# yuvalH9/UMERegRobust

Hardware: AMD Instinct MI355X
Metric: registration_pairs_per_s (higher is better)
Workload: dtype f32

## Files before the change

umeregrobust_amd/csrc/match_dev.h:

```cpp
#pragma once
#include "common.h"
#include "qlayout.h"

namespace umereg {

using f32x16 = __attribute__((ext_vector_type(16))) float;
using half8 = __attribute__((ext_vector_type(8))) _Float16;
using f32x2 = __attribute__((ext_vector_type(2))) float;

constexpr int kDistWaves = 4;

constexpr int kRegionCap = 512;
constexpr int kMaxSplits = 64;
constexpr unsigned int kShareMask = 0x8000808bu;

struct MatchScratch {
    unsigned int* rowlim;
    unsigned int* cnt;
    unsigned int* cand;
    int splits;
    unsigned int share_mask;
    int force_exhaustive;
    const int* ord1;
    const int* ord2;
    unsigned long long* stats;
};

constexpr int kCoarseTA = 2;
constexpr int kCoarseRows = kCoarseTA * 8;
constexpr int kCoarseWG = kCoarseRows * kDistWaves;

constexpr int kPK = 33;
constexpr int kPWaves = 8;
constexpr int kPRows = 32;
constexpr int kPWG = kPRows * kPWaves;
constexpr int kPRegionCap = 1024;

inline size_t qa_bytes(int n1) { return align_up((size_t)n1, 128) * 128 * sizeof(float); }
inline size_t qb_bytes(int n2) { return align_up((size_t)n2, 32) * 128 * sizeof(float); }
struct CoarsePlan {
    int n_ablk, n_blocks, n_btiles, splits, tiles_per_split;
    int sub_tiles, sub_tps, sub_splits;
};
struct MatchOpts {
    int variant = 0;
    int splits = 0;
    long long share_mask = -1;
    int exhaustive = 0;
};
inline int resolve_opts(const umereg_match_opts* o, MatchOpts& m, const char* who)
{
    m = MatchOpts();
    if (!o) return UMEREG_OK;
    UMEREG_REQUIRE(o->variant == 0 || o->variant == 1, "%s: unknown matcher variant %d (0 = Q-form, 1 = P-form)", who, (int)o->variant);
    UMEREG_REQUIRE(o->splits >= 0 && o->force_exhaustive >= 0, "%s: negative matcher option", who);
    UMEREG_REQUIRE(o->share_mask <= 0xffffffffll, "%s: share_mask does not fit 32 bits", who);
    UMEREG_REQUIRE(o->reserved == 0, "%s: umereg_match_opts.reserved must be 0 (got %d)", who, (int)o->reserved);
    m.variant = o->variant;
    m.splits = o->splits;
    m.share_mask = o->share_mask;
    m.exhaustive = o->force_exhaustive ? 1 : 0;
    return UMEREG_OK;
}
inline bool use_pform(const MatchOpts& o) { return o.variant == 1; }
constexpr int kNumCU = 256;
#ifndef UMEREG_COARSE_PHASES
#define UMEREG_COARSE_PHASES 3
#endif
constexpr int kMinSplitTiles = 4;
constexpr int kLeadMinTiles = 64;

inline CoarsePlan coarse_plan(int n1, int n2, const MatchOpts& o)
{
    CoarsePlan p;
    p.n_btiles = (n2 + 31) / 32;
    int splits;
    if (use_pform(o)) {
        p.n_ablk = (n1 + kPWG - 1) / kPWG;
        p.n_blocks = p.n_ablk * kPWaves;
        splits = kNumCU / p.n_ablk;
    } else {
        p.n_ablk = (n1 + kCoarseWG - 1) / kCoarseWG;
        p.n_blocks = p.n_ablk * kDistWaves;
        splits = (2560 + p.n_ablk - 1) / p.n_ablk;
    }
    p.sub_tiles = p.sub_tps = p.sub_splits = 0;
    if (UMEREG_COARSE_PHASES >= 2 && !use_pform(o) && o.splits <= 0 && p.n_btiles >= kLeadMinTiles) {
        const int n_sub = (n2 + kSubStride - 1) / kSubStride;
        p.sub_tiles = (n_sub + 31) / 32;
        int s1 = 4 * kNumCU / p.n_ablk;
        s1 = s1 < 1 ? 1 : (s1 > 16 ? 16 : s1);
        s1 = s1 > p.sub_tiles / kMinSplitTiles ? p.sub_tiles / kMinSplitTiles : s1;
        p.sub_tps = (p.sub_tiles + s1 - 1) / s1;
        p.sub_splits = (p.sub_tiles + p.sub_tps - 1) / p.sub_tps;
        const int bulk = p.n_btiles - p.sub_tiles;
        int s2 = splits > kMaxSplits - 16 ? kMaxSplits - 16 : splits;
        s2 = s2 > bulk / kMinSplitTiles ? bulk / kMinSplitTiles : s2;
        p.tiles_per_split = (bulk + s2 - 1) / s2;
        p.splits = p.sub_splits + (bulk + p.tiles_per_split - 1) / p.tiles_per_split;
        return p;
    }
    if (o.splits > 0) splits = o.splits;
    if (splits > kMaxSplits) splits = kMaxSplits;
    if (splits > p.n_btiles) splits = p.n_btiles;
    if (splits < 1) splits = 1;
    p.tiles_per_split = (p.n_btiles + splits - 1) / splits;
    p.splits = (p.n_btiles + p.tiles_per_split - 1) / p.tiles_per_split;
    return p;
}
inline size_t region_cap(const MatchOpts& o) { return use_pform(o) ? (size_t)kPRegionCap : (size_t)kRegionCap; }
inline size_t cand_bytes(int n1, const CoarsePlan& p, const MatchOpts& o)
{
    return align_up(((size_t)n1 + (size_t)p.n_blocks * p.splits * (1 + region_cap(o))) * sizeof(unsigned int), 256);
}
inline size_t pfrag_bytes(const CoarsePlan& p, const MatchOpts& o)
{
    return use_pform(o) ? ((size_t)p.n_blocks + (size_t)p.n_btiles) * kPK * 64 * sizeof(half8) : 0;
}
#ifndef UMEREG_COARSE_STATS
#define UMEREG_COARSE_STATS 0
#endif
constexpr size_t kStatsBytes = UMEREG_COARSE_STATS ? 256 : 0;
inline size_t match_scratch_bytes(int n1, int n2, const MatchOpts& o = MatchOpts())
{
    const CoarsePlan p = coarse_plan(n1, n2, o);
    return cand_bytes(n1, p, o) + pfrag_bytes(p, o) + kStatsBytes;
}

inline int match_args(const void* Q1_rows_h, const void* Q2_cols_h, int n1, int n2, void* scratch, size_t scratch_bytes,
                      const MatchOpts& o, const char* who)
{
    UMEREG_REQUIRE(Q1_rows_h && Q2_cols_h, "%s: null basis pointer", who);
    UMEREG_REQUIRE(n1 > 0 && n2 > 0, "%s: n1, n2 must be positive (got %d, %d)", who, n1, n2);
    UMEREG_REQUIRE(n2 < (1 << 27), "%s: n2 must be below 2^27 (got %d)", who, n2);
    UMEREG_REQUIRE(((uintptr_t)Q1_rows_h & 15) == 0 && ((uintptr_t)Q2_cols_h & 15) == 0, "%s: misaligned basis pointer", who);
    if (int rc = check_device()) return rc;
    if (!scratch || scratch_bytes < match_scratch_bytes(n1, n2, o) || ((uintptr_t)scratch & 15)) {
        set_error("%s: scratch too small or misaligned (%zu < %zu)", who, scratch_bytes, match_scratch_bytes(n1, n2, o));
        return UMEREG_EWORKSPACE;
    }
    return UMEREG_OK;
}

inline MatchScratch carve_scratch(void* scratch, int n1, const CoarsePlan& p, const MatchOpts& o, const int* ord1 = nullptr,
                                  const int* ord2 = nullptr)
{
    MatchScratch ms;
    ms.rowlim = (unsigned int*)scratch;
    ms.cnt = ms.rowlim + n1;
    ms.cand = ms.cnt + (size_t)p.n_blocks * p.splits;
    ms.splits = p.splits;
    ms.share_mask = o.share_mask >= 0 ? (unsigned int)o.share_mask : kShareMask;
    ms.force_exhaustive = o.exhaustive;
    ms.ord1 = ord1;
    ms.ord2 = ord2;
    ms.stats = UMEREG_COARSE_STATS ? (unsigned long long*)((char*)scratch + cand_bytes(n1, p, o) + pfrag_bytes(p, o)) : nullptr;
    return ms;
}
inline half8* pfrag_rows(void* scratch, int n1, const CoarsePlan& p, const MatchOpts& o) { return (half8*)((char*)scratch + cand_bytes(n1, p, o)); }
inline half8* pfrag_cols(void* scratch, int n1, const CoarsePlan& p, const MatchOpts& o) { return pfrag_rows(scratch, n1, p, o) + (size_t)p.n_blocks * kPK * 64; }

int launch_orthobasis_pair(const float* ume1, int n1, int layout1, float* Q1, const float* ume2, int n2, int layout2, float* Q2,
                           hipStream_t st, const int* order1 = nullptr, const int* order2 = nullptr);
int match_refine_f16(const void* Q1_rows_h, const void* Q2_cols_h, int n1, int n2, const void* scratch, size_t scratch_bytes,
                     int64_t* match_idx, float* match_dist, const umereg_match_opts* opts, const int* order1, const int* order2,
                     void* stream);
int match_f16r_ordered(const float* ume1, const float* ume2, int n1, int n2, const int* order1, const int* order2,
                       int64_t* match_idx, float* match_dist, void* workspace, size_t workspace_bytes,
                       const umereg_match_opts* opts, void* stream);

}
```

umeregrobust_amd/csrc/match_f16r.hip:

```cpp
#include <type_traits>

#include "common.h"
#include "match_dev.h"
#include "qlayout.h"

namespace umereg {

constexpr float kCoarseMargin = 0.03125f + 0.0009765625f;
constexpr float kCoarseTermMax = 1.00390625f;
#ifndef UMEREG_COARSE_EXIT
#define UMEREG_COARSE_EXIT 3
#endif

__device__ __forceinline__ float group32_max(float v)
{
    int x = __float_as_int(v);
    x = __float_as_int(fmaxf(__int_as_float(x), __int_as_float(__builtin_amdgcn_mov_dpp(x, 0xB1, 0xf, 0xf, true))));
    x = __float_as_int(fmaxf(__int_as_float(x), __int_as_float(__builtin_amdgcn_mov_dpp(x, 0x4E, 0xf, 0xf, true))));
    x = __float_as_int(fmaxf(__int_as_float(x), __int_as_float(__builtin_amdgcn_mov_dpp(x, 0x141, 0xf, 0xf, true))));
    x = __float_as_int(fmaxf(__int_as_float(x), __int_as_float(__builtin_amdgcn_mov_dpp(x, 0x140, 0xf, 0xf, true))));
    x = __float_as_int(fmaxf(__int_as_float(x), __int_as_float(__builtin_amdgcn_ds_swizzle(x, 0x401F))));
    return __int_as_float(x);
}

#ifndef UMEREG_COARSE_ABLATE
#define UMEREG_COARSE_ABLATE 0
#endif
#ifndef UMEREG_COARSE_TPS
#define UMEREG_COARSE_TPS 2
#endif
constexpr int kCoarseTPS = UMEREG_COARSE_TPS;

__global__ __launch_bounds__(kWave* kDistWaves, 2) void ume_coarse_h_kernel(
    const half8* __restrict__ Afrag, const half8* __restrict__ Bfrag, int n1, int n2, int n_ablk, int tile_lo, int tile_mid, int tile_hi,
    int lead_tps, int lead_splits, int tiles_per_split, int sp0, MatchScratch ms)
{
    __shared__ half8 ldsB[2][kCoarseTPS * 512];
    const int wave = __builtin_amdgcn_readfirstlane(threadIdx.x >> 6);
    const int lane = lane_id();
    const int ablk = blockIdx.x % n_ablk;
    const int spl = blockIdx.x / n_ablk;
    const int sp = sp0 + spl;
    const bool lead = spl < lead_splits;
    const int jt0 = lead ? tile_lo + spl * lead_tps : tile_mid + (spl - lead_splits) * tiles_per_split;
    const int jt1 = lead ? min(jt0 + lead_tps, tile_mid) : min(jt0 + tiles_per_split, tile_hi);
    const int h = lane >> 5;
    const int i_base = ablk * kCoarseWG + wave * kCoarseRows;

    half8 a[kCoarseTA][2];
#pragma unroll
    for (int t = 0; t < kCoarseTA; ++t)
#pragma unroll
        for (int s = 0; s < 2; ++s)
            a[t][s] = Afrag[((((size_t)(ablk * (kCoarseWG / 8) + wave * kCoarseTA + t)) * 2 + s) * 2 + 0) * 64 + lane];

    int lim[kCoarseTA][4];
    unsigned int seen[kCoarseTA][4];
#pragma unroll
    for (int t = 0; t < kCoarseTA; ++t)
#pragma unroll
        for (int g = 0; g < 4; ++g) {
            const int i = i_base + t * 8 + 2 * g + h;
            seen[t][g] = __hip_atomic_load(ms.rowlim + min(i, n1 - 1), __ATOMIC_RELAXED, __HIP_MEMORY_SCOPE_AGENT);
            lim[t][g] = i < n1 ? max(__float_as_int(1.0e-30f), (int)seen[t][g]) : __float_as_int(3.0e38f);
        }
#pragma unroll
    for (int t = 0; t < kCoarseTA; ++t)
#pragma unroll
        for (int s = 0; s < 2; ++s) asm volatile("" ::"v"(a[t][s]));

    const int blk = ablk * kDistWaves + wave;
    unsigned int* const region = ms.cand + ((size_t)blk * ms.splits + sp) * kRegionCap;
    int qn = 0;
    auto share = [&](bool reload) __attribute__((always_inline)) {
#pragma unroll
        for (int t = 0; t < kCoarseTA; ++t)
#pragma unroll
            for (int g = 0; g < 4; ++g) {
                const float v = group32_max(__int_as_float(lim[t][g]));
                const int i = i_base + t * 8 + 2 * g + h;
                if ((lane & 31) == 0 && i < n1 && __float_as_uint(v) > seen[t][g]) atomicMax(ms.rowlim + i, __float_as_uint(v));
                lim[t][g] = max(__float_as_int(v), (int)seen[t][g]);
            }
        if (reload) {
#pragma unroll
            for (int t = 0; t < kCoarseTA; ++t)
#pragma unroll
                for (int g = 0; g < 4; ++g) {
                    const int i = min(i_base + t * 8 + 2 * g + h, n1 - 1);
                    seen[t][g] = __hip_atomic_load(ms.rowlim + i, __ATOMIC_RELAXED, __HIP_MEMORY_SCOPE_AGENT);
                }
        }
    };

    half8 st[kCoarseTPS][2];
    const int c0 = threadIdx.x, c1 = 256 + threadIdx.x;
    const int src0 = ((c0 >> 6) * 2) * 64 + (c0 & 63), src1 = ((c1 >> 6) * 2) * 64 + (c1 & 63);
    auto gload = [&](int jg) __attribute__((always_inline)) {
#pragma unroll
        for (int q = 0; q < kCoarseTPS; ++q) {
            const int jt = min(jg + q, jt1 - 1);
            st[q][0] = Bfrag[(size_t)jt * 1024 + src0];
            st[q][1] = Bfrag[(size_t)jt * 1024 + src1];
        }
    };
    auto lstore = [&](int buf) __attribute__((always_inline)) {
#pragma unroll
        for (int q = 0; q < kCoarseTPS; ++q) {
            ldsB[buf][q * 512 + c0] = st[q][0];
            ldsB[buf][q * 512 + c1] = st[q][1];
        }
    };
    if (jt0 < jt1) {
        gload(jt0);
        lstore(0);
    }
    if (jt0 + kCoarseTPS < jt1) gload(jt0 + kCoarseTPS);
    __syncthreads();
    int cur = 0;
    auto share_point = [&](const int jt) __attribute__((always_inline)) {
        const int kt = jt - jt0;
        if ((ms.share_mask >> (kt < 31 ? kt : 31)) & 1u) {
            if (kt < 31 || (kt & 31) == 31) share(true);
        }
    };
#if UMEREG_COARSE_STATS
    unsigned int n_stop1 = 0, n_stop2 = 0;
#endif
    auto hopeless = [&](const float (&sc)[kCoarseTA][4], const int cols) __attribute__((always_inline)) {
        float d = sc[0][0] - __int_as_float(lim[0][0]);
#pragma unroll
        for (int t = 0; t < kCoarseTA; ++t)
#pragma unroll
            for (int g = 0; g < 4; ++g) d = fmaxf(d, sc[t][g] - __int_as_float(lim[t][g]));
        const bool stop = __builtin_amdgcn_ballot_w64(!(d < -(float)(4 - cols) * kCoarseTermMax)) == 0ull;
        return (UMEREG_COARSE_ABLATE & 16) ? true : stop;
    };
    auto filter = [&](const int jt, const float (&sc)[kCoarseTA][4]) __attribute__((always_inline)) {
        if (UMEREG_COARSE_ABLATE & 2) {
#pragma unroll
            for (int t = 0; t < kCoarseTA; ++t)
#pragma unroll
                for (int g = 0; g < 4; ++g) lim[t][g] = max(lim[t][g], __float_as_int(sc[t][g]));
            return;
        }
#pragma unroll
        for (int t = 0; t < kCoarseTA; ++t)
#pragma unroll
            for (int g = 0; g < 4; ++g) lim[t][g] = max(lim[t][g], __float_as_int(sc[t][g] - kCoarseMargin));
        share_point(jt);
        unsigned long long hit[kCoarseTA][4], any = 0;
#pragma unroll
        for (int t = 0; t < kCoarseTA; ++t)
#pragma unroll
            for (int g = 0; g < 4; ++g) {
                hit[t][g] = __builtin_amdgcn_ballot_w64(sc[t][g] >= __int_as_float(lim[t][g]));
                any |= hit[t][g];
            }
        if (__builtin_popcountll(any) > 8) {
#pragma unroll
            for (int t = 0; t < kCoarseTA; ++t)
#pragma unroll
                for (int g = 0; g < 4; ++g) lim[t][g] = __float_as_int(group32_max(__int_as_float(lim[t][g])));
            any = 0;
#pragma unroll
            for (int t = 0; t < kCoarseTA; ++t)
#pragma unroll
                for (int g = 0; g < 4; ++g) {
                    hit[t][g] = __builtin_amdgcn_ballot_w64(sc[t][g] >= __int_as_float(lim[t][g]));
                    any |= hit[t][g];
                }
        }
        if (any) {
            const unsigned int j = (unsigned int)(jt * 32 + (lane & 31));
#pragma unroll
            for (int t = 0; t < kCoarseTA; ++t)
#pragma unroll
                for (int g = 0; g < 4; ++g) {
                    const unsigned long long mask = hit[t][g];
                    if (mask) {
                        const int pos = qn + mbcnt(mask);
                        if (((mask >> lane) & 1ull) && pos < kRegionCap)
                            region[pos] = ((unsigned int)(t * 8 + 2 * g + h) << 27) | j;
                        qn += __builtin_popcountll(mask);
                    }
                }
        }
    };
    auto tile = [&](const int jt, const int q) __attribute__((always_inline)) {
        const half8* const lB = &ldsB[cur][q * 512];
        float sc[kCoarseTA][4];
        auto products = [&](const int b, f32x16 (&cc)[kCoarseTA]) __attribute__((always_inline)) {
            const half8 b0 = (UMEREG_COARSE_ABLATE & 8) ? a[0][0] : lB[(b * 2 + 0) * 64 + lane];
            const half8 b1 = (UMEREG_COARSE_ABLATE & 8) ? a[0][1] : lB[(b * 2 + 1) * 64 + lane];
            if (UMEREG_COARSE_ABLATE & 4) {
#pragma unroll
                for (int t = 0; t < kCoarseTA; ++t)
#pragma unroll
                    for (int e = 0; e < 16; ++e) cc[t][e] = (float)b0[e & 7] + (float)b1[(e + t) & 7];
            } else {
#pragma unroll
                for (int t = 0; t < kCoarseTA; ++t) cc[t] = __builtin_amdgcn_mfma_f32_32x32x16_f16(a[t][0], b0, f32x16{0}, 0, 0, 0);
#pragma unroll
                for (int t = 0; t < kCoarseTA; ++t) cc[t] = __builtin_amdgcn_mfma_f32_32x32x16_f16(a[t][1], b1, cc[t], 0, 0, 0);
            }
        };
        auto squares = [&](const int b, const f32x16 (&cc)[kCoarseTA]) __attribute__((always_inline)) {
#pragma unroll
            for (int t = 0; t < kCoarseTA; ++t)
#pragma unroll
                for (int g = 0; g < 4; ++g) {
                    if (UMEREG_COARSE_ABLATE & 1) {
                        sc[t][g] = b == 0 ? cc[t][4 * g] : sc[t][g] + cc[t][4 * g + 1];
                        continue;
                    }
                    float acc = b == 0 ? cc[t][4 * g] * cc[t][4 * g] : fmaf(cc[t][4 * g], cc[t][4 * g], sc[t][g]);
                    acc = fmaf(cc[t][4 * g + 1], cc[t][4 * g + 1], acc);
                    acc = fmaf(cc[t][4 * g + 2], cc[t][4 * g + 2], acc);
                    sc[t][g] = fmaf(cc[t][4 * g + 3], cc[t][4 * g + 3], acc);
                }
        };
        constexpr bool kTest1 = (UMEREG_COARSE_EXIT & 1) && !(UMEREG_COARSE_ABLATE & 15), kTest2 = (UMEREG_COARSE_EXIT & 2) && !(UMEREG_COARSE_ABLATE & 15);
        constexpr bool kAhead = (UMEREG_COARSE_EXIT & 4) != 0;
        f32x16 c0[kCoarseTA], c1[kCoarseTA];
        products(0, c0);
        if (kAhead || !kTest1) products(1, c1);
        squares(0, c0);
        if (kTest1 && hopeless(sc, 1)) {
#if UMEREG_COARSE_STATS
            ++n_stop1;
#endif
            share_point(jt);
            return;
        }
        if (!kAhead && kTest1) products(1, c1);
        squares(1, c1);
        if (kTest2 && hopeless(sc, 2)) {
#if UMEREG_COARSE_STATS
            ++n_stop2;
#endif
            share_point(jt);
            return;
        }
#pragma unroll
        for (int b = 2; b < 4; ++b) {
            f32x16 cc[kCoarseTA];
            products(b, cc);
            squares(b, cc);
        }
        filter(jt, sc);
    };
    for (int jg = jt0; jg < jt1; jg += kCoarseTPS) {
#pragma unroll
        for (int q = 0; q < kCoarseTPS; ++q)
            if (jg + q < jt1) tile(jg + q, q);
        if (jg + kCoarseTPS < jt1) lstore(cur ^ 1);
        if (jg + 2 * kCoarseTPS < jt1) gload(jg + 2 * kCoarseTPS);
        __syncthreads();
        cur ^= 1;
    }
    share(false);
    if (lane == 0) ms.cnt[(size_t)blk * ms.splits + sp] = (unsigned int)qn;
#if UMEREG_COARSE_STATS
    if (lane == 0) {
        atomicAdd(ms.stats + 0, (unsigned long long)max(jt1 - jt0, 0));
        atomicAdd(ms.stats + 1, (unsigned long long)n_stop1);
        atomicAdd(ms.stats + 2, (unsigned long long)n_stop2);
        atomicAdd(ms.stats + 3, (unsigned long long)qn);
    }
#endif
}

constexpr float kCoarseMarginP = 0.009765625f;
constexpr int kPDepth = 5;
constexpr int kQsStride = 33;

__global__ __launch_bounds__(256) void pform_pack_kernel(const _Float16* __restrict__ Ah, const _Float16* __restrict__ Bh, int n1,
                                                         int n2, int tiles1, int tiles2, half8* __restrict__ PA,
                                                         half8* __restrict__ PB)
{
    __shared__ float4 qs[32 * kQsStride];
    const int side = blockIdx.y, tile = blockIdx.x;
    if (tile >= (side ? tiles2 : tiles1)) return;
    const int n = side ? n2 : n1;
    const _Float16* const Q = side ? Bh : Ah;
    half8* const P = (side ? PB : PA) + (size_t)tile * kPK * 64;
    const int tid = threadIdx.x;
    if (tile * 32 >= n) {
        for (int o = tid; o < kPK * 64; o += 256) P[o] = half8{0};
        return;
    }
    float* const qf = reinterpret_cast<float*>(qs);
    for (int c = tid; c < 512; c += 256) {
        const int kp = c & 31, a = (c >> 5) & 3, k8 = c >> 7;
        const int i = tile * 32 + kp;
        half8 vh = half8{0}, vl = half8{0};
        if (i < n) {
            const size_t off0 = side ? hoff_cols(i, a, k8 * 8, 0) : hoff_rows(i, a, k8 * 8, 0);
            const size_t off1 = side ? hoff_cols(i, a, k8 * 8, 1) : hoff_rows(i, a, k8 * 8, 1);
            vh = *reinterpret_cast<const half8*>(Q + off0);
            vl = *reinterpret_cast<const half8*>(Q + off1);
        }
#pragma unroll
        for (int x = 0; x < 8; ++x) qf[(kp * kQsStride + k8 * 8 + x) * 4 + a] = (float)vh[x] + (float)vl[x];
    }
    __syncthreads();
    for (int o = tid; o < kPK * 64; o += 256) {
        const int ks = o >> 6, l = o & 63, kp = l & 31, c = ks * 2 + (l >> 5);
        half8 out = half8{0};
        if (c < 66) {
            const int d = c < 64 ? c >> 2 : 16, u0 = c < 64 ? (c & 3) * 8 : (c - 64) * 8;
            const float w = d == 0 ? 1.0f : 1.41421356237f;
#pragma unroll
            for (int e = 0; e < 8; ++e) {
                const float4 qu = qs[kp * kQsStride + u0 + e], qv = qs[kp * kQsStride + ((u0 + e + d) & 31)];
                out[e] = (_Float16)(w * fmaf(qu.x, qv.x, fmaf(qu.y, qv.y, fmaf(qu.z, qv.z, qu.w * qv.w))));
            }
        }
        P[o] = out;
    }
}

__global__ __launch_bounds__(kWave* kPWaves, 2) void ume_coarse_p_kernel(const half8* __restrict__ PA, const half8* __restrict__ PB,
                                                                        int n1, int n2, int n_ablk, int n_btiles,
                                                                        int tiles_per_split, MatchScratch ms)
{
    __shared__ half8 ldsB[3][kPK * 64];
    __shared__ __attribute__((aligned(16))) unsigned int seenL[kPWaves][32];
    const int wave = __builtin_amdgcn_readfirstlane(threadIdx.x >> 6);
    const int lane = lane_id();
    const int ablk = blockIdx.x % n_ablk;
    const int sp = blockIdx.x / n_ablk;
    const int jt0 = sp * tiles_per_split;
    const int jt1 = min(jt0 + tiles_per_split, n_btiles);
    const int h = lane >> 5;
    const int atile = ablk * kPWaves + wave;
    const int i_base = atile * 32;

    half8 a[kPK];
#pragma unroll
    for (int ks = 0; ks < kPK; ++ks) a[ks] = PA[((size_t)atile * kPK + ks) * 64 + lane];

    int lim[16];
#pragma unroll
    for (int r = 0; r < 16; ++r) {
        const int i = i_base + (r >> 2) * 8 + h * 4 + (r & 3);
        lim[r] = __float_as_int(i < n1 ? 1.0e-30f : 3.0e38f);
    }
    int qn = 0;
    auto fetch_seen = [&]() __attribute__((always_inline)) {
        if (lane < 32)
            __builtin_amdgcn_global_load_lds((const __attribute__((address_space(1))) void*)(ms.rowlim + min(i_base + lane, n1 - 1)),
                                             (__attribute__((address_space(3))) void*)(&seenL[wave][0]), 4, 0, 16 );
    };
    auto share = [&](bool reload) __attribute__((always_inline)) {
        asm volatile("s_waitcnt vmcnt(0)" ::: "memory");
#pragma unroll
        for (int g = 0; g < 4; ++g) {
            const uint4 sv = *reinterpret_cast<const uint4*>(&seenL[wave][g * 8 + h * 4]);
            const unsigned int seen[4] = {sv.x, sv.y, sv.z, sv.w};
#pragma unroll
            for (int e = 0; e < 4; ++e) {
                const int r = g * 4 + e;
                const float v = group32_max(__int_as_float(lim[r]));
                const int i = i_base + g * 8 + h * 4 + e;
                if ((lane & 31) == 0 && i < n1 && __float_as_uint(v) > seen[e]) atomicMax(ms.rowlim + i, __float_as_uint(v));
                lim[r] = max(__float_as_int(v), (int)seen[e]);
            }
        }
        if (reload) fetch_seen();
    };
    unsigned int* const region = ms.cand + ((size_t)atile * ms.splits + sp) * kPRegionCap;
    auto tile_candidates = [&](const f32x16& cc, const int jt) __attribute__((always_inline)) {
        unsigned long long any = 0;
#pragma unroll
        for (int r = 0; r < 16; ++r) any |= __builtin_amdgcn_ballot_w64(cc[r] >= __int_as_float(lim[r]));
        if (__builtin_popcountll(any) > 8) {
#pragma unroll
            for (int r = 0; r < 16; ++r) lim[r] = __float_as_int(group32_max(__int_as_float(lim[r])));
        }
        const unsigned int j = (unsigned int)(jt * 32 + (lane & 31));
#pragma unroll
        for (int r = 0; r < 16; ++r) {
            const unsigned long long mask = __builtin_amdgcn_ballot_w64(cc[r] >= __int_as_float(lim[r]));
            if (mask) {
                const int pos = qn + mbcnt(mask);
                if (((mask >> lane) & 1ull) && pos < kPRegionCap)
                    region[pos] = ((unsigned int)((r >> 2) * 8 + h * 4 + (r & 3)) << 27) | j;
                qn += __builtin_popcountll(mask);
            }
        }
    };

    auto stage = [&](int jt, int buf) __attribute__((always_inline)) {
        const half8* const src = PB + (size_t)jt * kPK * 64 + lane;
#pragma unroll
        for (int q = 0; q < (kPK + kPWaves / 2 - 1) / (kPWaves / 2); ++q) {
            const int f = q * (kPWaves / 2) + wave;
            if (f < kPK)
                __builtin_amdgcn_global_load_lds((const __attribute__((address_space(1))) void*)(src + f * 64),
                                                 (__attribute__((address_space(3))) void*)(&ldsB[buf][f * 64]), 16, 0, 0);
        }
    };
    auto limits = [&](const f32x16& cc, unsigned int& fl) __attribute__((always_inline)) {
#pragma unroll
        for (int r = 0; r < 16; ++r) {
            lim[r] = max(lim[r], __float_as_int(cc[r] - kCoarseMarginP));
            fl = __builtin_amdgcn_alignbit(fl, __float_as_int(cc[r] - __int_as_float(lim[r])), 31);
        }
    };
    auto bookkeeping = [&](const f32x16& cc, const unsigned int fl, const int jp) __attribute__((always_inline)) {
        const int kt = jp - jt0;
        if ((ms.share_mask >> (kt < 31 ? kt : 31)) & 1u) {
            if (kt < 31 || (kt & 31) == 31) share(true);
        }
        unsigned int hits = ~fl & 0xffffu;
        unsigned long long mask = __builtin_amdgcn_ballot_w64(hits != 0);
        if (__builtin_popcountll(mask) > 8) {
            tile_candidates(cc, jp);
        } else {
            const unsigned int j = (unsigned int)(jp * 32 + (lane & 31));
            while (mask) {
                if (hits) {
                    const int k = 31 - __builtin_clz(hits);
                    hits &= ~(1u << k);
                    const int r = 15 - k;
                    const int pos = qn + mbcnt(mask);
                    if (pos < kPRegionCap) region[pos] = ((unsigned int)((r >> 2) * 8 + h * 4 + (r & 3)) << 27) | j;
                }
                qn += __builtin_popcountll(mask);
                mask = __builtin_amdgcn_ballot_w64(hits != 0);
            }
        }
    };
    auto mfma_panel = [&](const int buf, f32x16& acc, const f32x16& prev, unsigned int& fl, auto interleave) __attribute__((always_inline)) {
        const half8* const lb = &ldsB[buf][lane];
        half8 b[kPDepth];
#pragma unroll
        for (int q = 0; q < kPDepth; ++q) b[q] = lb[q * 64];
        __builtin_amdgcn_sched_barrier(0);
#pragma unroll
        for (int ks = 0; ks < kPK; ++ks) {
            if (ks >= 1 && ks - 1 + kPDepth < kPK) b[(ks - 1) % kPDepth] = lb[(ks - 1 + kPDepth) * 64];
            __builtin_amdgcn_sched_barrier(0);
            if (ks == 0) asm volatile("v_mfma_f32_32x32x16_f16 %0, %1, %2, 0" : "=v"(acc) : "a"(a[ks]), "v"(b[ks % kPDepth]));
            else if (ks < 32) asm volatile("v_mfma_f32_32x32x16_f16 %0, %1, %2, %0" : "+v"(acc) : "a"(a[ks]), "v"(b[ks % kPDepth]));
            else asm volatile("v_mfma_f32_32x32x16_f16 %0, %1, %2, %0" : "+v"(acc) : "v"(a[ks]), "v"(b[ks % kPDepth]));
            if (decltype(interleave)::value && ks < 32 && (ks & 1) == 0) {
                const int r = ks >> 1;
                lim[r] = max(lim[r], __float_as_int(prev[r] - kCoarseMarginP));
                fl = __builtin_amdgcn_alignbit(fl, __float_as_int(prev[r] - __int_as_float(lim[r])), 31);
                asm volatile("" : "+v"(fl), "+v"(lim[r]));
            }
            __builtin_amdgcn_sched_barrier(0);
        }
        asm volatile("s_nop 15\n\ts_nop 15\n\ts_nop 15\n\ts_nop 15" : "+v"(acc) : : "memory");
    };
    const bool young = wave >= kPWaves / 2;
    auto panel = [&](const int jt, f32x16& acc, f32x16& prev) __attribute__((always_inline)) {
        const int buf = (jt - jt0) % 3;
        unsigned int fl = ~0u;
        if (young) {
            if (jt > jt0) {
                limits(prev, fl);
                bookkeeping(prev, fl, jt - 1);
            }
            mfma_panel(buf, acc, prev, fl, std::false_type{});
        } else {
            mfma_panel(buf, acc, prev, fl, std::true_type{});
            asm volatile("s_waitcnt vmcnt(0)" ::: "memory");
            if (jt > jt0) bookkeeping(prev, fl, jt - 1);
            if (jt + 2 < jt1) stage(jt + 2, (buf + 2) % 3);
        }
        asm volatile("s_waitcnt lgkmcnt(0)\n\ts_barrier" ::: "memory");
    };
    if (!young) {
        if (jt0 < jt1) stage(jt0, 0);
        if (jt0 + 1 < jt1) stage(jt0 + 1, 1);
    }
    fetch_seen();
    asm volatile("s_waitcnt vmcnt(0)" ::: "memory");
    __syncthreads();
    f32x16 accA, accB;
    accA = accB = f32x16{-1.0f};
    int jt = jt0;
    for (; jt + 1 < jt1; jt += 2) {
        panel(jt, accA, accB);
        panel(jt + 1, accB, accA);
    }
    if (jt < jt1) {
        panel(jt, accA, accB);
        accB = accA;
    }
    if (jt0 < jt1) {
        unsigned int fl = ~0u;
        limits(accB, fl);
        bookkeeping(accB, fl, jt1 - 1);
    }
    share(false);
    if (lane == 0) ms.cnt[(size_t)atile * ms.splits + sp] = (unsigned int)qn;
}

constexpr int kQiStride = 130;

template <int kRows, int kCap>
__global__ __launch_bounds__(256, 4) void match_refine_kernel(const _Float16* __restrict__ Ah,
                                                           const _Float16* __restrict__ Bh, int n1, int n2,
                                                           MatchScratch ms, int64_t* __restrict__ idx,
                                                           float* __restrict__ dist)
{
    constexpr int kCoarseRows = kRows, kRegionCap = kCap;
    __shared__ double qi[kCoarseRows * kQiStride];
    __shared__ unsigned long long best[kCoarseRows];
    __shared__ unsigned int offs[kWave + 1];
    __shared__ int overflow;
    const int blk = blockIdx.x;
    const int i0 = blk * kCoarseRows;
    const int tid = threadIdx.x;
    if (tid < kWave) {
        const unsigned int c = tid < ms.splits ? ms.cnt[(size_t)blk * ms.splits + tid] : 0u;
        const bool ovf = c > (unsigned int)kRegionCap;
        unsigned int incl = min(c, (unsigned int)kRegionCap);
#pragma unroll
        for (int d = 1; d < kWave; d <<= 1) {
            const unsigned int up = (unsigned int)__shfl_up((int)incl, d, kWave);
            if (tid >= d) incl += up;
        }
        offs[tid + 1] = incl;
        const bool any_ovf = __builtin_amdgcn_ballot_w64(ovf) != 0ull;
        if (tid == 0) {
            offs[0] = 0;
            overflow = any_ovf || ms.force_exhaustive;
        }
    }
    if (tid < kCoarseRows) best[tid] = ~0ull;
    for (int e = tid; e < kCoarseRows * 16; e += blockDim.x) {
        const int r = e >> 4, a = (e >> 2) & 3, k8 = e & 3;
        const int i = min(i0 + r, n1 - 1);
        const half8 vh = *reinterpret_cast<const half8*>(Ah + hoff_rows(i, a, k8 * 8, 0));
        const half8 vl = *reinterpret_cast<const half8*>(Ah + hoff_rows(i, a, k8 * 8, 1));
#pragma unroll
        for (int x = 0; x < 8; ++x) qi[r * kQiStride + (k8 * 8 + x) * 4 + a] = (double)vh[x] + (double)vl[x];
    }
    __syncthreads();
    const bool exhaustive = overflow != 0;
    const unsigned int total = exhaustive ? (unsigned int)kCoarseRows * (unsigned int)n2 : offs[ms.splits];
    const unsigned int* const regions = ms.cand + (size_t)blk * ms.splits * kRegionCap;
    int sp = 0;
    for (unsigned int e = tid; e < total; e += blockDim.x) {
        unsigned int r, j;
        if (exhaustive) {
            r = e % kCoarseRows;
            j = e / kCoarseRows;
        } else {
            while (e >= offs[sp + 1]) ++sp;
            const unsigned int ent = regions[(size_t)sp * kRegionCap + (e - offs[sp])];
            r = ent >> 27;
            j = ent & 0x07ffffffu;
        }
        const double* const q = qi + r * kQiStride;
        double dot[4][4];
#pragma unroll
        for (int a = 0; a < 4; ++a)
#pragma unroll
            for (int b = 0; b < 4; ++b) dot[a][b] = 0.0;
#pragma unroll 2
        for (int k8 = 0; k8 < 4; ++k8) {
            half8 vh[4], vl[4];
#pragma unroll
            for (int b = 0; b < 4; ++b) {
                vh[b] = *reinterpret_cast<const half8*>(Bh + hoff_cols((int)j, b, k8 * 8, 0));
                vl[b] = *reinterpret_cast<const half8*>(Bh + hoff_cols((int)j, b, k8 * 8, 1));
            }
#pragma unroll
            for (int x = 0; x < 8; ++x) {
                const int k = k8 * 8 + x;
                const double q0 = q[k * 4 + 0], q1 = q[k * 4 + 1], q2 = q[k * 4 + 2], q3 = q[k * 4 + 3];
#pragma unroll
                for (int b = 0; b < 4; ++b) {
                    const double v = (double)((float)vh[b][x] + (float)vl[b][x]);
                    dot[0][b] = fma(q0, v, dot[0][b]);
                    dot[1][b] = fma(q1, v, dot[1][b]);
                    dot[2][b] = fma(q2, v, dot[2][b]);
                    dot[3][b] = fma(q3, v, dot[3][b]);
                }
            }
        }
        double s = 0.0;
#pragma unroll
        for (int a = 0; a < 4; ++a)
#pragma unroll
            for (int b = 0; b < 4; ++b) s = fma(dot[a][b], dot[a][b], s);
        const float d2 = (float)fmax(4.0 - s, 0.0);
        if (d2 == d2 && (int)(i0 + r) < n1) {
            const unsigned int jk = ms.ord2 ? (unsigned int)ms.ord2[target_slot_pos((int)j, n2)] : j;
            atomicMin(&best[r], ((unsigned long long)__float_as_uint(d2) << 32) | jk);
        }
    }
    __syncthreads();
    if (tid < kCoarseRows && i0 + tid < n1) {
        const unsigned long long k = best[tid];
        const bool ok = k != ~0ull;
        const int ik = ms.ord1 ? ms.ord1[i0 + tid] : i0 + tid;
        idx[ik] = ok ? (int64_t)(unsigned int)(k & 0xffffffffull) : 0;
        if (dist) dist[ik] = ok ? sqrtf(__uint_as_float((unsigned int)(k >> 32))) : 2.0f;
    }
}

}

using namespace umereg;

UMEREG_API int umereg_ume_match_coarse_f16_ex(const void* Q1_rows_h, const void* Q2_cols_h, int n1, int n2, void* scratch,
                                              size_t scratch_bytes, const umereg_match_opts* opts, void* stream)
{
    MatchOpts o;
    if (int rc = resolve_opts(opts, o, "ume_match_coarse_f16")) return rc;
    if (int rc = match_args(Q1_rows_h, Q2_cols_h, n1, n2, scratch, scratch_bytes, o, "ume_match_coarse_f16")) return rc;
    hipStream_t st = (hipStream_t)stream;
    const CoarsePlan p = coarse_plan(n1, n2, o);
    const MatchScratch ms = carve_scratch(scratch, n1, p, o);
    if (use_pform(o)) {
        half8* const PA = pfrag_rows(scratch, n1, p, o);
        half8* const PB = pfrag_cols(scratch, n1, p, o);
        const int tiles = p.n_blocks > p.n_btiles ? p.n_blocks : p.n_btiles;
        hipLaunchKernelGGL(pform_pack_kernel, dim3(tiles, 2), dim3(256), 0, st, (const _Float16*)Q1_rows_h, (const _Float16*)Q2_cols_h,
                           n1, n2, p.n_blocks, p.n_btiles, PA, PB);
        UMEREG_CHECK_LAUNCH("pform_pack_kernel");
        hipLaunchKernelGGL(ume_coarse_p_kernel, dim3(p.n_ablk * p.splits), dim3(kWave * kPWaves), 0, st, PA, PB, n1, n2, p.n_ablk,
                           p.n_btiles, p.tiles_per_split, ms);
        UMEREG_CHECK_LAUNCH("ume_coarse_p_kernel");
        return UMEREG_OK;
    }
    const dim3 wg(kWave * kDistWaves);
    if (p.sub_tiles && UMEREG_COARSE_PHASES == 2) {
        hipLaunchKernelGGL(ume_coarse_h_kernel, dim3(p.n_ablk * p.sub_splits), wg, 0, st, (const half8*)Q1_rows_h, (const half8*)Q2_cols_h,
                           n1, n2, p.n_ablk, 0, p.sub_tiles, p.sub_tiles, p.sub_tps, p.sub_splits, 1, 0, ms);
        UMEREG_CHECK_LAUNCH("ume_coarse_h_kernel");
        hipLaunchKernelGGL(ume_coarse_h_kernel, dim3(p.n_ablk * (p.splits - p.sub_splits)), wg, 0, st, (const half8*)Q1_rows_h,
                           (const half8*)Q2_cols_h, n1, n2, p.n_ablk, p.sub_tiles, p.sub_tiles, p.n_btiles, 1, 0, p.tiles_per_split,
                           p.sub_splits, ms);
    } else {
        hipLaunchKernelGGL(ume_coarse_h_kernel, dim3(p.n_ablk * p.splits), wg, 0, st, (const half8*)Q1_rows_h, (const half8*)Q2_cols_h,
                           n1, n2, p.n_ablk, 0, p.sub_tiles, p.n_btiles, p.sub_tiles ? p.sub_tps : 1, p.sub_splits, p.tiles_per_split, 0, ms);
    }
    UMEREG_CHECK_LAUNCH("ume_coarse_h_kernel");
    return UMEREG_OK;
}
UMEREG_API int umereg_ume_match_coarse_f16(const void* Q1_rows_h, const void* Q2_cols_h, int n1, int n2, void* scratch,
                                           size_t scratch_bytes, void* stream)
{
    return umereg_ume_match_coarse_f16_ex(Q1_rows_h, Q2_cols_h, n1, n2, scratch, scratch_bytes, nullptr, stream);
}

int umereg::match_refine_f16(const void* Q1_rows_h, const void* Q2_cols_h, int n1, int n2, const void* scratch, size_t scratch_bytes,
                             int64_t* match_idx, float* match_dist, const umereg_match_opts* opts, const int* order1,
                             const int* order2, void* stream)
{
    UMEREG_REQUIRE(match_idx, "ume_match_refine_f16: null match_idx");
    MatchOpts o;
    if (int rc = resolve_opts(opts, o, "ume_match_refine_f16")) return rc;
    if (int rc = match_args(Q1_rows_h, Q2_cols_h, n1, n2, (void*)scratch, scratch_bytes, o, "ume_match_refine_f16")) return rc;
    const CoarsePlan p = coarse_plan(n1, n2, o);
    const MatchScratch ms = carve_scratch((void*)scratch, n1, p, o, order1, order2);
    if (use_pform(o))
        hipLaunchKernelGGL((match_refine_kernel<kPRows, kPRegionCap>), dim3(p.n_blocks), dim3(256), 0, (hipStream_t)stream,
                           (const _Float16*)Q1_rows_h, (const _Float16*)Q2_cols_h, n1, n2, ms, match_idx, match_dist);
    else
        hipLaunchKernelGGL((match_refine_kernel<kCoarseRows, kRegionCap>), dim3(p.n_blocks), dim3(256), 0, (hipStream_t)stream,
                           (const _Float16*)Q1_rows_h, (const _Float16*)Q2_cols_h, n1, n2, ms, match_idx, match_dist);
    UMEREG_CHECK_LAUNCH("match_refine_kernel");
    return UMEREG_OK;
}
UMEREG_API int umereg_ume_match_refine_f16_ex(const void* Q1_rows_h, const void* Q2_cols_h, int n1, int n2,
                                              const void* scratch, size_t scratch_bytes, int64_t* match_idx,
                                              float* match_dist, const umereg_match_opts* opts, void* stream)
{
    return match_refine_f16(Q1_rows_h, Q2_cols_h, n1, n2, scratch, scratch_bytes, match_idx, match_dist, opts, nullptr, nullptr, stream);
}
UMEREG_API int umereg_ume_match_refine_f16(const void* Q1_rows_h, const void* Q2_cols_h, int n1, int n2,
                                           const void* scratch, size_t scratch_bytes, int64_t* match_idx,
                                           float* match_dist, void* stream)
{
    return umereg_ume_match_refine_f16_ex(Q1_rows_h, Q2_cols_h, n1, n2, scratch, scratch_bytes, match_idx, match_dist, nullptr, stream);
}
```

Baseline: 3946.

## Stage coarse B tiles via direct global-to-LDS loads and raise occupancy

Replaces the register-staged global load plus LDS store double buffer in the coarse matcher with global_load_lds_dwordx4 inline asm that writes B fragments straight into LDS. A triple buffer is used when one tile is processed per step. Launch bounds rise from 2 to 4 blocks per CU, freeing the registers that held staged data. The lead split count now comes from the occupancy query at runtime. This removes VGPR staging and lets loads overlap compute. The risks are hand-written waitcnt and barrier sequencing, and register spilling under the tighter bound.

```diff
diff --git a/umeregrobust_amd/csrc/match_dev.h b/umeregrobust_amd/csrc/match_dev.h
--- a/umeregrobust_amd/csrc/match_dev.h
+++ b/umeregrobust_amd/csrc/match_dev.h
@@ -70,6 +70,9 @@
 constexpr int kMinSplitTiles = 4;
 constexpr int kLeadMinTiles = 64;
 
+constexpr int kCoarseResidentBuilt = 4;
+int coarse_resident_per_cu();
+
 inline CoarsePlan coarse_plan(int n1, int n2, const MatchOpts& o)
 {
     CoarsePlan p;
@@ -88,7 +91,7 @@
     if (UMEREG_COARSE_PHASES >= 2 && !use_pform(o) && o.splits <= 0 && p.n_btiles >= kLeadMinTiles) {
         const int n_sub = (n2 + kSubStride - 1) / kSubStride;
         p.sub_tiles = (n_sub + 31) / 32;
-        int s1 = 4 * kNumCU / p.n_ablk;
+        int s1 = coarse_resident_per_cu() * kNumCU / p.n_ablk;
         s1 = s1 < 1 ? 1 : (s1 > 16 ? 16 : s1);
         s1 = s1 > p.sub_tiles / kMinSplitTiles ? p.sub_tiles / kMinSplitTiles : s1;
         p.sub_tps = (p.sub_tiles + s1 - 1) / s1;
diff --git a/umeregrobust_amd/csrc/match_f16r.hip b/umeregrobust_amd/csrc/match_f16r.hip
--- a/umeregrobust_amd/csrc/match_f16r.hip
+++ b/umeregrobust_amd/csrc/match_f16r.hip
@@ -30,12 +30,13 @@
 #define UMEREG_COARSE_TPS 2
 #endif
 constexpr int kCoarseTPS = UMEREG_COARSE_TPS;
-
-__global__ __launch_bounds__(kWave* kDistWaves, 2) void ume_coarse_h_kernel(
+constexpr int kCoarseBufs = kCoarseTPS == 1 ? 3 : 2;
+
+__global__ __launch_bounds__(kWave* kDistWaves, 4) void ume_coarse_h_kernel(
     const half8* __restrict__ Afrag, const half8* __restrict__ Bfrag, int n1, int n2, int n_ablk, int tile_lo, int tile_mid, int tile_hi,
     int lead_tps, int lead_splits, int tiles_per_split, int sp0, MatchScratch ms)
 {
-    __shared__ half8 ldsB[2][kCoarseTPS * 512];
+    __shared__ half8 ldsB[kCoarseBufs][kCoarseTPS * 512];
     const int wave = __builtin_amdgcn_readfirstlane(threadIdx.x >> 6);
     const int lane = lane_id();
     const int ablk = blockIdx.x % n_ablk;
@@ -93,30 +94,28 @@
         }
     };
 
-    half8 st[kCoarseTPS][2];
-    const int c0 = threadIdx.x, c1 = 256 + threadIdx.x;
-    const int src0 = ((c0 >> 6) * 2) * 64 + (c0 & 63), src1 = ((c1 >> 6) * 2) * 64 + (c1 & 63);
-    auto gload = [&](int jg) __attribute__((always_inline)) {
+    auto stage = [&](int jg, int buf) __attribute__((always_inline)) {
 #pragma unroll
         for (int q = 0; q < kCoarseTPS; ++q) {
             const int jt = min(jg + q, jt1 - 1);
-            st[q][0] = Bfrag[(size_t)jt * 1024 + src0];
-            st[q][1] = Bfrag[(size_t)jt * 1024 + src1];
-        }
-    };
-    auto lstore = [&](int buf) __attribute__((always_inline)) {
-#pragma unroll
-        for (int q = 0; q < kCoarseTPS; ++q) {
-            ldsB[buf][q * 512 + c0] = st[q][0];
-            ldsB[buf][q * 512 + c1] = st[q][1];
-        }
-    };
-    if (jt0 < jt1) {
-        gload(jt0);
-        lstore(0);
-    }
-    if (jt0 + kCoarseTPS < jt1) gload(jt0 + kCoarseTPS);
-    __syncthreads();
+#pragma unroll
+            for (int r = 0; r < 2; ++r) {
+                const int run = r * kDistWaves + wave;
+                const unsigned int dst = (unsigned int)(uintptr_t)(__attribute__((address_space(3))) void*)(&ldsB[buf][q * 512 + run * 64]);
+                asm volatile("s_mov_b32 m0, %0\n\ts_nop 0\n\tglobal_load_lds_dwordx4 %1, off"
+                             :: "s"(dst), "v"(Bfrag + (size_t)jt * 1024 + run * 128 + lane) : "memory");
+            }
+        }
+    };
+    auto group_end = [&](const bool ahead) __attribute__((always_inline)) {
+        if (kCoarseBufs == 3 && ahead) asm volatile("s_waitcnt vmcnt(%0)" ::"n"(2 * kCoarseTPS) : "memory");
+        else asm volatile("s_waitcnt vmcnt(0)" ::: "memory");
+        asm volatile("s_waitcnt lgkmcnt(0)\n\ts_barrier" ::: "memory");
+    };
+#pragma unroll
+    for (int g = 0; g < kCoarseBufs - 1; ++g)
+        if (jt0 + g * kCoarseTPS < jt1) stage(jt0 + g * kCoarseTPS, g);
+    group_end(kCoarseBufs == 3 && jt0 + kCoarseTPS < jt1);
     int cur = 0;
     auto share_point = [&](const int jt) __attribute__((always_inline)) {
         const int kt = jt - jt0;
@@ -251,13 +250,13 @@
         filter(jt, sc);
     };
     for (int jg = jt0; jg < jt1; jg += kCoarseTPS) {
+        const bool ahead = jg + (kCoarseBufs - 1) * kCoarseTPS < jt1;
+        if (ahead) stage(jg + (kCoarseBufs - 1) * kCoarseTPS, cur == 0 ? kCoarseBufs - 1 : cur - 1);
 #pragma unroll
         for (int q = 0; q < kCoarseTPS; ++q)
             if (jg + q < jt1) tile(jg + q, q);
-        if (jg + kCoarseTPS < jt1) lstore(cur ^ 1);
-        if (jg + 2 * kCoarseTPS < jt1) gload(jg + 2 * kCoarseTPS);
-        __syncthreads();
-        cur ^= 1;
+        group_end(ahead);
+        cur = cur + 1 == kCoarseBufs ? 0 : cur + 1;
     }
     share(false);
     if (lane == 0) ms.cnt[(size_t)blk * ms.splits + sp] = (unsigned int)qn;
@@ -610,6 +609,19 @@
 }
 
 using namespace umereg;
+
+int umereg::coarse_resident_per_cu()
+{
+    static const int resident = [] {
+        int n = 0;
+        if (hipOccupancyMaxActiveBlocksPerMultiprocessor(&n, ume_coarse_h_kernel, kWave * kDistWaves, 0) != hipSuccess) {
+            (void)hipGetLastError();
+            return kCoarseResidentBuilt;
+        }
+        return n < 1 ? 1 : (n > 8 ? 8 : n);
+    }();
+    return resident;
+}
 
 UMEREG_API int umereg_ume_match_coarse_f16_ex(const void* Q1_rows_h, const void* Q2_cols_h, int n1, int n2, void* scratch,
                                               size_t scratch_bytes, const umereg_match_opts* opts, void* stream)
```

Result: slower. 3817 (-3.3%).
